# wkh923/m3pc

Hardware: AMD Instinct MI355X
Metric: MPC plan-steps/sec (N=1024, H=16, hopper-medium-v2); independent plan steps, 3 in flight (higher is better)
Workload: dtype bf16; 1 GPU; hopper-medium-v2 shapes (S=11,A=3) rtg_guiding N=1024 H=16 T=32 bf16 candidate pass + fp32 policy pass + fp32 re-score (arg-max and multinomial draw certified under the calibrated bound delta, 8.4 candidates re-scored on average); 3 independent plan steps in flight (policy pass / candidate pass / re-score of neighbouring steps on different streams); window resident in HBM; candidates_per_gpu=1024, global_candidates=1024, horizon=16, traj_length=32, steps_in_flight=3, settle_steps=24, parallelism=1 GPU

## Files before the change

include/m3pc_hip_debug.h:

```cpp
#ifndef M3PC_HIP_DEBUG_H
#define M3PC_HIP_DEBUG_H

#ifdef __cplusplus
extern "C" {
#endif

int m3pc_debug_gemm(int dtype, const void* A, const void* Wt, const float* bias, const float* res, void* C, int M, int N,
                    int K, int gelu, int f32out, int variant, void* stream);
typedef struct m3pc_debug_gemm_args {
    int dtype;
    const void* A;
    int lda;
    int amap[3];
    const void* W;
    int ldw;
    int M, N, K;
    const float* bias;
    const float* rowtab;
    int rt_mod, rt_ld;
    int gelu;
    const float* res;
    int ldr;
    void* C;
    int f32out;
// ... 553 lines not shown
    const float* grad;
    long long grad_floats;
    float* exp_avg;
    float* exp_avg_sq;
    long long state_floats;
    const long long* steps_in;
    long long* steps_out;
    int write_bf16;
    double lr_t, weight_decay, beta1, beta2, eps;
    void* stream;
    int* n_blocks;
} m3pc_debug_mtm_adamw_args;
int m3pc_debug_mtm_adamw(const m3pc_debug_mtm_adamw_args* a);
int m3pc_debug_stamp_log(m3pc_handle* h, int cap, long long* out, int* n_logged);
int m3pc_debug_step_streams_created(m3pc_handle* h);
int m3pc_debug_xcc_probe(int* out, int n_blocks, void* stream);

#ifdef __cplusplus
}
#endif
#endif
```

m3pc_amd/csrc/elementwise.hip:

```cpp
#include "device_util.h"

namespace m3pc {

#ifdef M3PC_LAB
thread_local int g_ew_picked = 0;
#endif

__global__ __launch_bounds__(256) void embed_kernel(EmbedP p) {
    const long long row = blockIdx.x;
    const int b = (int)(row / p.L), j = (int)(row % p.L);
    const int2 kt = p.tokmap[j];
    const int key = kt.x, t = kt.y;
    const int D = p.feat[key];
    const float* x = p.tok[key] + (long long)b * p.bstride[key] + (p.widx ? (long long)p.widx[b] * p.wstride[key] : 0) + (long long)t * D;
    __shared__ float xs[32];
    if (threadIdx.x < D) {
        float v = x[threadIdx.x];
        if (p.normalize[key]) v = (v - p.mean[key][threadIdx.x]) / p.stdv[key][threadIdx.x];
        xs[threadIdx.x] = v;
    }
    __syncthreads();
    const float* WT = p.WT[key];
    const float* E = p.E[key] + (long long)t * p.d;
    float* out = p.X + row * p.d;
// ... 104 lines not shown
                for (int i = 0; i < NV; ++i) {
                    const float c0 = x[i].x - mean, c1 = x[i].y - mean, c2 = x[i].z - mean, c3 = x[i].w - mean;
                    q += (c0 * c0 + c1 * c1) + (c2 * c2 + c3 * c3);
                }
                const float rstd = rsqrtf(wave_sum(q) / (float)d + 1e-5f);
#pragma unroll
                for (int i = 0; i < NV; ++i) {
                    y[i].x = (x[i].x - mean) * rstd * gv[i].x + bv[i].x;
                    y[i].y = (x[i].y - mean) * rstd * gv[i].y + bv[i].y;
                    y[i].z = (x[i].z - mean) * rstd * gv[i].z + bv[i].z;
                    y[i].w = (x[i].w - mean) * rstd * gv[i].w + bv[i].w;
                }
            }
        }
        const long long row = (long long)b * p.L + j;
        if (!(indep && p.x_first_only && b > 0)) {
            if (p.Xb) {
                const long long xrow = p.x_compact ? block_res_row_xb((int)row, p.L, p.n_indep) : row;
#pragma unroll
                for (int i = 0; i < NV; ++i) {
                    bf16x4 o;
                    o[0] = (bf16_t)x[i].x;
                    o[1] = (bf16_t)x[i].y;
                    o[2] = (bf16_t)x[i].z;
                    o[3] = (bf16_t)x[i].w;
                    stream_store(o, (bf16x4*)(p.Xb + xrow * d + (i * 64 + lane) * 4));
                }
            } else {
#pragma unroll
                for (int i = 0; i < NV; ++i) *(float4*)(p.X + row * d + (i * 64 + lane) * 4) = x[i];
            }
        }
        if (!p.ln_g) continue;
        if (p.Hf) {
#pragma unroll
            for (int i = 0; i < NV; ++i) *(float4*)(p.Hf + row * d + (i * 64 + lane) * 4) = y[i];
        }
        if (p.Hb) {
            bf16_t* dst;
            if (p.n_sh == 0)
                dst = p.Hb + row * d;
            else if (j >= p.n_sh)
                dst = p.Hb + ((long long)b * n_own + (j - p.n_sh)) * d;
            else if (b == 0)
                dst = p.Hb_sh + (long long)j * d;
            else
                continue;
#pragma unroll
            for (int i = 0; i < NV; ++i) {
                bf16x4 o;
                o[0] = (bf16_t)y[i].x;
                o[1] = (bf16_t)y[i].y;
                o[2] = (bf16_t)y[i].z;
                o[3] = (bf16_t)y[i].w;
                stream_store(o, (bf16x4*)(dst + (i * 64 + lane) * 4));
            }
        }
    }
}
// ... 851 lines not shown
```

m3pc_amd/csrc/kernels.h:

```cpp
#pragma once
#include <hip/hip_runtime.h>
#include <stdint.h>

#ifdef M3PC_LAB
#define M3PC_ENV(name) getenv(name)
#else
#define M3PC_ENV(name) ((const char*)nullptr)
#endif

namespace m3pc {

typedef __bf16 bf16_t;

enum DType { DT_F32 = 0, DT_BF16 = 1, DT_X3 = 2 };

static inline size_t dtype_size(int dt) { return dt == DT_F32 ? 4 : 2; }

#ifndef M3PC_STREAM_AUX
#define M3PC_STREAM_AUX 0
#endif
template <typename V>
__device__ __forceinline__ V stream_load(const V* p) { return M3PC_STREAM_AUX ? __builtin_nontemporal_load(p) : *p; }
template <typename V>
__device__ __forceinline__ void stream_store(V v, V* p) {
// ... 245 lines not shown
    const float* E[4];
    int feat[4];
    const int2* tokmap;
    int batch, L, d, T;
    float* X;
    bf16_t* Xb;
    const float* ln_g;
    const float* ln_b;
    float* Hf;
    bf16_t* Hb;
    int n_indep;
    int x_first_only;
    int x_compact;
    int n_sh;
    bf16_t* Hb_sh;
};
void launch_embed(const EmbedP& p, hipStream_t st);

struct GatherP {
    const float* Xe;
    long long xe_bstride;
    const float* table;
    const int* rowsrc;
    int rows_per_batch, batch, d;
    float* out;
    bf16_t* outb;
};
void launch_gather_rows(const GatherP& p, hipStream_t st);

struct HeadOutP {
// ... 246 lines not shown
```

m3pc_amd/csrc/m3pc.hip:

```cpp
#include "m3pc_internal.h"
#include "mtm_loss.h"

namespace m3pc {
thread_local char g_err[512] = "";
int fail(int code, const char* fmt, ...) {
    va_list ap;
    va_start(ap, fmt);
    vsnprintf(g_err, sizeof(g_err), fmt, ap);
    va_end(ap);
    return code;
}
}

namespace {

int find_tensor(const m3pc_named_tensor* list, int n, const std::string& name) {
    for (int i = 0; i < n; ++i)
        if (list[i].name && name == list[i].name) return i;
    return -1;
}


}

// ... 64 lines not shown
        }
        if (is_dirty("mask_token_dict." + kn))
            HIPCHK(hipMemcpyAsync(h->mask_tokens + (size_t)k * d, W(h, "mask_token_dict." + kn).f, d * sizeof(float),
                                  hipMemcpyDeviceToDevice, st));
    }
    bool dec_dirty = pos_dirty;
    for (const std::string& nme : dirty)
        if (nme.rfind("decoder", 0) == 0 || nme.rfind("mask_token_dict", 0) == 0) dec_dirty = true;
    if (dec_dirty) {
        invalidate_tables(h);
        ls[3] = 1;
    }
    for (int sl = 0; sl < M3PC_SLOTS; ++sl) {
        h->slot[sl].policy_valid = false;
        h->slot[sl].n_windows = 0;
    }
    return 0;
}
}

#pragma GCC visibility push(default)
extern "C" {

const char* m3pc_last_error(void) { return g_err; }
int m3pc_abi_version(void) { return M3PC_ABI_VERSION; }

int m3pc_create(const m3pc_dims* dims, int device, m3pc_handle** out) {
    if (!dims || !out) return fail(M3PC_EINVAL, "null argument");
    const m3pc_dims& D = *dims;
    if (D.n_embd % 64 || D.n_embd > 1024 || D.n_head <= 0 || D.n_embd % D.n_head)
// ... 164 lines not shown
        hipFree(h->Edec[k]);
        hipFree(h->tok_mean[k]);
        hipFree(h->tok_std[k]);
    }
    hipFree(h->mask_tokens);
    mtm_loss_free(h);
    free_ws(h->base);
    for (int par = 0; par < 2; ++par) {
        free_ws(h->chain[par]);
        free_ws(h->pchain[par]);
    }
    for (int s = 0; s < M3PC_SLOTS; ++s) {
        hipFree(h->slot[s].loc);
        hipFree(h->slot[s].sd);
        hipFree(h->slot[s].rtok);
    }
    void* bufs[] = {h->sel_scratch, h->d_topk, h->er_top, h->sa_buf, h->sa_chain[0], h->sa_chain[1], h->c_om, h->c_os, h->goal_ws,
                    h->refine_noise, h->refine_scores, h->refine_elites, h->refine_widx};
    for (int s = 0; s < M3PC_SLOTS; ++s) {
        void* cb[] = {h->cert_list[s], h->cert_b[s], h->cert_f[s], h->cert_stats[s], h->cert_f32[s], h->cert_top1[s]};
        for (void* b : cb)
            if (b) hipFree(b);
        for (int i = 0; i < 4; ++i)
            if (h->step_ev[s][i]) hipEventDestroy(h->step_ev[s][i]);
    }
    if (h->ev_excl) hipEventDestroy(h->ev_excl);
    if (h->step_chain_own)
        for (int i = 0; i < 2; ++i)
            if (h->step_chain[i]) hipStreamDestroy(h->step_chain[i]);
    if (h->cert_host) hipHostFree(h->cert_host);
// ... 80 lines not shown
    if (!h || !out4) return fail(M3PC_EINVAL, "null argument");
    for (int i = 0; i < 4; ++i) out4[i] = h->load_stats[i];
    return 0;
}

int m3pc_set_tokenizer(m3pc_handle* h, int key, const float* mean, const float* std_, int dim, int normalize) {
    if (!h || key < 0 || key > 3 || !mean || !std_) return fail(M3PC_EINVAL, "bad argument");
    if (dim != h->feat[key]) return fail(M3PC_EINVAL, "tokenizer '%s' has dim %d, expected %d", KEYN[key], dim, h->feat[key]);
    HIPCHK(hipSetDevice(h->device));
    HIPCHK(hipMemcpy(h->tok_mean[key], mean, dim * sizeof(float), hipMemcpyHostToDevice));
    HIPCHK(hipMemcpy(h->tok_std[key], std_, dim * sizeof(float), hipMemcpyHostToDevice));
    h->h_mean[key].assign(mean, mean + dim);
    h->h_std[key].assign(std_, std_ + dim);
    h->tok_norm[key] = normalize ? 1 : 0;
    h->tok_set[key] = true;
    return 0;
}

int m3pc_set_critic(m3pc_handle* h, const m3pc_named_tensor* tensors, int n, const float* obs_mean, const float* obs_std,
                    void* stream) {
    if (!h || !tensors || !obs_mean || !obs_std) return fail(M3PC_EINVAL, "null argument");
    if (h->dm.critic_hidden <= 0) return fail(M3PC_EINVAL, "handle was created without a critic");
    hipStream_t st = (hipStream_t)stream;
    HIPCHK(hipSetDevice(h->device));
    HIPCHK(hipStreamSynchronize(st));
    const int Hd = h->dm.critic_hidden, SA = h->S + h->A;
    auto fetch = [&](const std::string& name, long long numel, std::vector<float>& out) -> int {
        const int i = find_tensor(tensors, n, name);
        if (i < 0) return fail(M3PC_EINVAL, "critic state_dict is missing '%s'", name.c_str());
        if (tensors[i].numel != numel) return fail(M3PC_EINVAL, "'%s' has %lld elements, expected %lld", name.c_str(), tensors[i].numel, numel);
// ... 254 lines not shown
    if (a->mode < 0 || a->mode > 2) return fail(M3PC_EINVAL, "bad mode %d", a->mode);
    if (!precision_ok(a->precision)) return fail(M3PC_EINVAL, "bad precision %d", a->precision);
    if (a->slot < 0 || a->slot >= M3PC_SLOTS) return fail(M3PC_EINVAL, "slot %d outside [0, %d)", a->slot, M3PC_SLOTS);
    if (a->flags & ~(M3PC_PLAN_DEFER_JOIN | M3PC_PLAN_PRUNED_POLICY))
        return fail(M3PC_EINVAL, "unknown m3pc_plan_args::flags 0x%x (is the caller's structure the ABI v%d one?)", a->flags, M3PC_ABI_VERSION);
    if (need_critic && a->mode != M3PC_MODE_RTG && !h->critic_set) return fail(M3PC_ESTATE, "critic weights not set");
    HIPCHK(hipSetDevice(h->device));
    bind_slot(h, a->slot);
    return 0;
}

int m3pc_policy_pass(m3pc_handle* h, const m3pc_plan_args* a, const float* states, const float* actions, const float* rewards,
                     float* loc, float* std_, void* stream) {
    if (!h || !a || !states || !actions || !rewards) return fail(M3PC_EINVAL, "null argument");
    CHK(plan_check(h, a, false));
    hipStream_t st = (hipStream_t)stream;
    const int T = h->T, hh = a->horizon, idx = T - hh;
    if (a->returns) {
        launch_tokenize(a->returns, a->returns_f64, h->rtok, T, 1, h->tok_mean[M3PC_RETURNS], h->tok_std[M3PC_RETURNS],
                        h->tok_norm[M3PC_RETURNS], st);
    } else {
        double rt = a->rtg;
        if (h->tok_norm[M3PC_RETURNS]) rt = (rt - (double)h->h_mean[M3PC_RETURNS][0]) / (double)h->h_std[M3PC_RETURNS][0];
        launch_fill(h->rtok, (float)rt, T, st);
    }
    Plan* pl = nullptr;
    CHK(get_mask_plan(h, 0, idx, &pl));
    TokIn in;
    memset(&in, 0, sizeof(in));
    in.ptr[M3PC_STATES] = states;
// ... 98 lines not shown
        sp.n_begin = a->n_begin + c0;
        sp.n_count = cnt;
        sp.cand = h->base.cand + (size_t)c0 * T * h->A;
        sp.sample_actions = sample_actions + (size_t)c0 * hh * h->A;
        if (c0 == 0) {
            sp.loc_out = loc;
            sp.sd_out = std_;
        }
        launch_sample(sp, s);
    };

    const int dt = pass_dt(a->precision);
    X3Scope x3(h, a->precision == M3PC_PREC_BF16X3);
    const int n = a->n_count;
    h->slot_join_n[a->slot] = 0;
    if (h->two_stream && dt == DT_BF16 && n >= 512 && (long long)n * (2 * T - hh + 1) > 256 * 128) {
        std::vector<int> parts;
        if (!h->stream_split.empty()) {
            int left = n;
            for (int v : h->stream_split)
                if (v > 0 && v < left && parts.size() + 1 < h->auxs.size() + 1) {
                    parts.push_back(v);
                    left -= v;
                }
            parts.push_back(left);
        } else {
            int n0 = ((n / 2 + 127) / 128) * 128;
            parts = {n0, n - n0};
        }
        const bool defer = (a->flags & M3PC_PLAN_DEFER_JOIN) != 0 && !h->prof_serial && parts.size() <= 4;
// ... 44 lines not shown
    for (int i = 0; i < h->slot_join_n[slot]; ++i) HIPCHK(hipStreamWaitEvent((hipStream_t)stream, h->slot_join[slot][i], 0));
    h->slot_join_n[slot] = 0;
    return 0;
}

int m3pc_plan_step(m3pc_handle* h, const m3pc_plan_args* a, const float* states, const float* actions, const float* rewards,
                   const float* eps, float* loc, float* std_, float* sample_actions, float* expect_return,
                   float* pred_rewards, float* pred_boot, void* stream) {
    if (!h || !a || !states || !actions || !rewards || !eps || !sample_actions || !expect_return)
        return fail(M3PC_EINVAL, "null argument");
    if (a->mode >= 0 && a->mode <= 2 && a->mode != M3PC_MODE_RTG && !h->critic_set) return fail(M3PC_ESTATE, "critic weights not set");
    if (a->n_count < 1 || a->n_begin < 0 || a->n_begin + a->n_count > a->n_total)
        return fail(M3PC_EINVAL, "candidate range [%d,+%d) outside n_total=%d", a->n_begin, a->n_count, a->n_total);
    if (a->n_count > h->dm.max_candidates) return fail(M3PC_ENOMEM, "n_count %d > max_candidates %d", a->n_count, h->dm.max_candidates);
    CHK(m3pc_policy_pass(h, a, states, actions, rewards, nullptr, nullptr, stream));
    return m3pc_candidate_pass(h, a, states, actions, rewards, eps, loc, std_, sample_actions, expect_return, pred_rewards,
                               pred_boot, stream);
}

static int fill_rtok(m3pc_handle* h, const double* rtg, int n_windows, hipStream_t st) {
    for (int w = 0; w < n_windows; ++w) {
        double rt = rtg[w];
        if (h->tok_norm[M3PC_RETURNS]) rt = (rt - (double)h->h_mean[M3PC_RETURNS][0]) / (double)h->h_std[M3PC_RETURNS][0];
        launch_fill(h->rtok + (size_t)w * h->T, (float)rt, h->T, st);
    }
    return 0;
}

int m3pc_score_actions(m3pc_handle* h, const m3pc_plan_args* a, int n_windows, const float* states, const float* actions,
                       const float* rewards, const float* cand, const int* window_index, float* expect_return,
// ... 64 lines not shown
    in.normalize[M3PC_ACTIONS] = h->tok_norm[M3PC_ACTIONS];
    in.ptr[M3PC_REWARDS] = rewards;
    in.bstride[M3PC_REWARDS] = T;
    in.normalize[M3PC_REWARDS] = h->tok_norm[M3PC_REWARDS];
    in.ptr[M3PC_RETURNS] = h->rtok;
    in.bstride[M3PC_RETURNS] = T;
    h->allow_splitk = true;
    {
        WsScope ws(h, true, true, a->slot);
        const int rc = forward_impl(h, pl, in, E, nullptr, nullptr, nullptr, h->loc, h->sd, DT_F32, st);
        h->allow_splitk = false;
        if (rc) return rc;
    }
    h->slot[a->slot].policy_valid = E == 1;
    h->slot[a->slot].n_windows = E;
    if (loc) HIPCHK(hipMemcpyAsync(loc, h->loc, (size_t)E * T * A * sizeof(float), hipMemcpyDeviceToDevice, st));
    if (std_) HIPCHK(hipMemcpyAsync(std_, h->sd, (size_t)E * T * A * sizeof(float), hipMemcpyDeviceToDevice, st));
    return check_launch("policy_pass_batch");
}

int m3pc_plan_step_batch(m3pc_handle* h, const m3pc_plan_args* a, int n_windows, const float* states, const float* actions,
                         const float* rewards, const double* rtg, const float* eps, const int* window_index, float* loc,
                         float* std_, float* sample_actions, float* expect_return, void* stream) {
    if (!h || !a || !states || !actions || !rewards || !rtg || !eps || !window_index || !sample_actions || !expect_return)
        return fail(M3PC_EINVAL, "null argument");
    const int T = h->T, E = n_windows, N = a->n_total;
    if (!precision_ok(a->precision)) return fail(M3PC_EINVAL, "bad precision %d", a->precision);
    if (E >= 1 && (N < 1 || (long long)E * N > h->dm.max_candidates))
        return fail(M3PC_ENOMEM, "n_windows * n_total = %lld > max_candidates %d", (long long)E * N, h->dm.max_candidates);
    if (a->mode >= 0 && a->mode <= 2 && a->mode != M3PC_MODE_RTG && !h->critic_set) return fail(M3PC_ESTATE, "critic weights not set");
// ... 513 lines not shown
```

m3pc_amd/csrc/m3pc_certified.hip:

```cpp
#include <atomic>
#include <chrono>

#include "m3pc_internal.h"

namespace m3pc {
int cert_check_args(const m3pc_plan_args* a, const char* who) {
    if (a->n_total < 1 || a->n_total > 16384) return fail(M3PC_EINVAL, "%s: n_total %d outside [1, 16384]", who, a->n_total);
    if (a->n_begin != 0 || a->n_count != a->n_total)
        return fail(M3PC_EINVAL, "%s plans on one rank: candidates [%d,+%d) are not all n_total=%d", who, a->n_begin, a->n_count, a->n_total);
    if (!precision_ok(a->precision)) return fail(M3PC_EINVAL, "bad precision %d", a->precision);
    if (a->slot < 0 || a->slot >= M3PC_SLOTS) return fail(M3PC_EINVAL, "slot %d outside [0, %d)", a->slot, M3PC_SLOTS);
    return 0;
}
bool cert_any_begun(const m3pc_handle* h) {
    for (int s = 0; s < M3PC_SLOTS; ++s)
        if (h->cstep[s].begun) return true;
    return false;
}
}

#pragma GCC visibility push(default)
extern "C" {

static int cert_wait_blocks(const volatile float* hs, const float* dev, const float* seq, int n, int n_device, hipStream_t st, float* out) {
// ... 233 lines not shown
    if (with_eval && !(eval_tol > 0.f)) return fail(M3PC_EINVAL, "%s: eval_tol must be > 0 (+inf: report only)", who);
    if (cert_any_begun(h)) return fail(M3PC_ESTATE, "%s with a pipelined step begun (m3pc_plan_step_certified_end first)", who);
    memset(rec, 0, sizeof(*rec));
    if (with_eval) {
        memset(erec, 0, sizeof(*erec));
        if (a->precision != M3PC_PREC_FP32) CHK(eval_host_setup(h));
    }
    CertStep& S = h->cstep[a->slot];
    cert_fill(S, a, c, states, actions, rewards, eps, expo, sample_actions, scores_low, merged, list, p, eval_action, argmax, sample_idx,
              sample_action, (hipStream_t)stream, false, with_eval ? eval_tol : 0.f);

    m3pc_plan_args pa = *a;
    pa.flags = a->flags & M3PC_PLAN_PRUNED_POLICY;
    pa.window = 0;
    CHK(m3pc_policy_pass(h, &pa, states, actions, rewards, nullptr, nullptr, stream));
    pa.flags = 0;
    CHK(m3pc_candidate_pass(h, &pa, states, actions, rewards, eps, loc, std_, sample_actions, scores_low, nullptr, nullptr, stream));
    CHK(cert_first_pass(h, S));
    return cert_resolve_step(h, S, rec, with_eval ? erec : nullptr);
}

int m3pc_plan_step_certified(m3pc_handle* h, const m3pc_plan_args* a, const m3pc_cert_args* c, const float* states, const float* actions,
                             const float* rewards, const float* eps, const float* expo, float* loc, float* std_, float* sample_actions,
                             float* scores_low, float* merged, int* list, float* p, float* eval_action, int* argmax, int* sample_idx,
                             float* sample_action, m3pc_cert_record* rec, void* stream) {
    return cert_step_serial(h, a, c, states, actions, rewards, eps, expo, loc, std_, sample_actions, scores_low, merged, list, p, eval_action,
                            argmax, sample_idx, sample_action, rec, false, 0.f, nullptr, stream, "m3pc_plan_step_certified");
}

int m3pc_plan_step_certified_eval(m3pc_handle* h, const m3pc_plan_args* a, const m3pc_cert_args* c, const float* states,
// ... 66 lines not shown
    CertStep& S = h->cstep[slot];
    if (S.begun) return fail(M3PC_ESTATE, "%s: the step in slot %d has not been ended", who, slot);
    HIPCHK(hipSetDevice(h->device));
    CHK(step_setup(h));
    if (with_eval && a->precision != M3PC_PREC_FP32) CHK(eval_host_setup(h));
    hipStream_t st = (hipStream_t)stream, chain = h->step_chain[slot & 1];
    hipEvent_t* ev = h->step_ev[slot];
    if (!(a->flags & M3PC_PLAN_INPUTS_READY)) {
        HIPCHK(hipEventRecord(ev[0], st));
        HIPCHK(hipStreamWaitEvent(chain, ev[0], 0));
    }
    m3pc_plan_args pa = *a;
    pa.flags = a->flags & M3PC_PLAN_PRUNED_POLICY;
    pa.window = 0;
    CHK(m3pc_policy_pass(h, &pa, states, actions, rewards, nullptr, nullptr, chain));
    HIPCHK(hipEventRecord(ev[1], chain));
    for (;;) {
        int o = -1;
        for (int s = 0; s < M3PC_SLOTS; ++s)
            if ((s & 1) == (slot & 1) && h->cstep[s].begun && h->cstep[s].tail_pending && (o < 0 || h->cstep[s].order < h->cstep[o].order))
                o = s;
        if (o < 0) break;
        CHK(step_enqueue_tail(h, o));
    }
    HIPCHK(hipStreamWaitEvent(st, ev[1], 0));
    if (h->excl_valid) HIPCHK(hipStreamWaitEvent(st, h->ev_excl, 0));
    if (h->cand_last_slot >= 0) HIPCHK(hipStreamWaitEvent(st, h->step_ev[h->cand_last_slot][2], 0));
    pa.flags = M3PC_PLAN_DEFER_JOIN;
    CHK(m3pc_candidate_pass(h, &pa, states, actions, rewards, eps, loc, std_, sample_actions, scores_low, nullptr, nullptr, stream));
    HIPCHK(hipEventRecord(ev[2], st));
// ... 435 lines not shown
```

m3pc_amd/csrc/m3pc_debug.hip:

```cpp
#include "m3pc_internal.h"
#include "mtm_grad.h"
#include "iql.h"
#include "mtm_opt.h"

#include <vector>

#pragma GCC visibility push(default)
extern "C" {

int m3pc_debug_step_streams_created(m3pc_handle* h) { return h ? h->step_streams_created : -1; }
int m3pc_debug_gemm(int dtype, const void* A, const void* Wt, const float* bias, const float* res, void* C, int M, int N,
                    int K, int gelu, int f32out, int variant, void* stream) {
    static const int ldpad = M3PC_ENV("M3PC_DEBUG_LDPAD") ? atoi(M3PC_ENV("M3PC_DEBUG_LDPAD")) : 0;
    GemmP p = gemm_basic(A, K + ldpad, Wt, K + ldpad, M, N, K, bias);
    p.a_padded = 0;
    p.gelu = gelu;
    p.res = res;
    p.ldr = N;
    p.variant = variant;
    if (dtype == DT_BF16 && !f32out)
        p.Cb = (bf16_t*)C;
    else
        p.Cf = (float*)C;
    p.ldc = N;
    if (dtype != DT_BF16 && variant != 1) {
// ... 1897 lines not shown
```

m3pc_amd/csrc/m3pc_internal.h:

```cpp
#pragma once
#include <math.h>
#include <stdarg.h>
#include <stdio.h>
#include <stdlib.h>
#include <string.h>

#include <algorithm>
#include <map>
#include <mutex>
#include <memory>
#include <string>
#include <vector>

#include "../../include/m3pc_hip.h"
#ifdef M3PC_LAB
#include "../../include/m3pc_hip_debug.h"
#endif
#include "cert_resolve.h"
#include "kernels.h"
#include "mtm_batch.h"

using namespace m3pc;

namespace m3pc {
// ... 151 lines not shown
    } ls;
    hipStream_t step_chain[2] = {nullptr, nullptr};
    bool step_chain_own = false;
    int step_streams_created = 0;
    hipEvent_t step_ev[M3PC_SLOTS][4] = {};
    hipEvent_t ev_excl = nullptr;
    bool excl_valid = false;
    int cand_last_slot = -1;
    unsigned long long step_order = 0;
    struct Slot {
        float *loc = nullptr, *sd = nullptr, *rtok = nullptr;
        bool policy_valid = false;
        int n_windows = 0;
    } slot[M3PC_SLOTS];
    int cur_slot = 0;
    struct Base {
        float *X = nullptr, *Y = nullptr, *EncOut = nullptr, *G = nullptr, *cand = nullptr, *pred[2] = {nullptr, nullptr},
              *qv = nullptr, *splitk_ws = nullptr;
        char *Hn = nullptr, *QKV = nullptr, *O = nullptr, *F = nullptr, *Z = nullptr;
        long long splitk_ws_bytes = 0;
        float* head_part = nullptr;
        int* head_ticket = nullptr;
        int head_rows = 0;
        long long R = 0;
        int max_cand = 0;
    } base, chain[2], pchain[2];
    Base* cur = nullptr;
    bool two_stream = true;
    bool allow_splitk = true;
    bool x3 = false;
// ... 320 lines not shown
    g.rowsrc = rowsrc;
    g.rows_per_batch = rows_per_batch;
    g.batch = batch;
    g.d = h->d;
    return g;
}

struct PassSwitches {
    bool no_block_fused;
    bool no_block_split;
    bool no_qkv_fused;
    bool no_fused_anything;
    bool no_prune1;
    bool no_bf16_residual;
    bool no_shared_xb;
    bool no_kv_fused;
    bool no_mix_prefix;
    bool no_head_fused;
    bool no_head_out_mfma;
    bool no_head_f32_fused;
    bool no_group;
};
inline const PassSwitches& pass_switches() {
    static const PassSwitches s = [] {
        auto on = [](const char* v) { return v != nullptr; };
        PassSwitches w{};
        w.no_block_fused = on(M3PC_ENV("M3PC_NO_BLOCK_FUSED"));
        w.no_block_split = on(M3PC_ENV("M3PC_NO_BLOCK_SPLIT"));
        w.no_qkv_fused = on(M3PC_ENV("M3PC_NO_QKV_FUSED"));
        w.no_fused_anything = w.no_block_fused || w.no_qkv_fused;
        w.no_prune1 = on(M3PC_ENV("M3PC_NO_PRUNE1"));
        w.no_bf16_residual = on(M3PC_ENV("M3PC_NO_BF16_RESIDUAL"));
        w.no_shared_xb = on(M3PC_ENV("M3PC_NO_SHARED_XB"));
        w.no_kv_fused = on(M3PC_ENV("M3PC_NO_KV_FUSED")) || w.no_block_fused;
        w.no_mix_prefix = on(M3PC_ENV("M3PC_NO_MIX_PREFIX"));
        w.no_head_fused = on(M3PC_ENV("M3PC_NO_HEAD_FUSED"));
        w.no_head_out_mfma = on(M3PC_ENV("M3PC_NO_HEAD_OUT_MFMA"));
        const bool no_f32_direct = on(M3PC_ENV("M3PC_NO_F32_DIRECT"));
        w.no_head_f32_fused = on(M3PC_ENV("M3PC_NO_HEAD_F32_FUSED")) || no_f32_direct;
        w.no_group = on(M3PC_ENV("M3PC_NO_GEMM_GROUP")) || no_f32_direct || on(M3PC_ENV("M3PC_GEMM_VARIANT"));
        return w;
    }();
    return s;
}

constexpr long long FUSED_MIN_ROWS = 96 * 128;
constexpr long long SPLIT_MIN_ROWS = 16 * 128;

struct PieceState {
    bool ln = true, qkv = false;
};

struct BlockArgs {
    const std::string& pfx;
    float* X;
    int batch, L;
    int n_sh = 0;
    const LnP* next_ln = nullptr;
    bool x_dead = false;
    const std::string* next_qkv = nullptr;
    bool x_bf16 = false;
    float* Xnext = nullptr;
    int res_nshared = 0;
};

struct TokIn {
    const float* ptr[4];
    long long bstride[4];
    int normalize[4];
    const int* widx = nullptr;
    long long wstride[4] = {0, 0, 0, 0};
};

enum { TAIL_HEADS = 0, TAIL_X = 1 };

int get_plan(m3pc_handle* h, const unsigned char* const masks[4], Plan** out);
int get_mask_plan(m3pc_handle* h, int kind, int idx, Plan** out);
int ensure_edec(m3pc_handle* h, Plan* pl, hipStream_t st);
// ... 9 lines not shown
int run_encoder(m3pc_handle* h, Plan* pl, const TokIn& in, int batch, int dt, hipStream_t st, bool bf16_out_only = false,
                int n_indep = 0, int layer_from = 0, int layer_to = 1 << 30, PieceState* ln_state = nullptr);
void dec_embed(m3pc_handle* h, int k, const void* Zop, RowMap amap, float* Yout, RowMap cmap, int M, int mod, int dt,
               hipStream_t st, const float* table = nullptr);
int run_decoder_full(m3pc_handle* h, const void* Zop, int batch, int dt, hipStream_t st);
int run_head(m3pc_handle* h, int k, const float* Ysrc, RowMap xmap, int rows, float* out, int ldy, bool detok, int dt,
             hipStream_t st);
int run_head_tail(m3pc_handle* h, int k, const void* ln_rows, int rows, float* out, int ldy, bool detok, int dt, hipStream_t st);
int forward_impl(m3pc_handle* h, Plan* pl, const TokIn& in, int batch, float* out_states, float* out_rewards,
                 float* out_returns, float* out_mu, float* out_std, int dt, hipStream_t st);
int pruned_decoder(m3pc_handle* h, Plan* pl, Plan::Query& q, SharedTables& tb, int n, int dt, hipStream_t st, int tail,
                   float** xrows);
int candidate_pass(m3pc_handle* h, const m3pc_plan_args* a, const float* states, const float* rewards, int n,
                   const float* sample_actions, float* expect_return, float* pred_rewards, float* pred_boot, int dt,
                   hipStream_t st, const int* widx = nullptr, int stage_from = 0, int stage_to = 1 << 30, PieceState* ln_state = nullptr);

}
```

m3pc_amd/csrc/m3pc_passes.hip:

```cpp
#include "m3pc_internal.h"

namespace m3pc {

struct TailRes {
    const float* rows = nullptr;
    const float* table = nullptr;
    int mod = 0;
    int nu = 0;
};

static bool chain_tail(m3pc_handle* h, const std::string& pfx, int rows, int dt, hipStream_t st, const TailRes& res, float* Xout,
                       const LnP* next_ln) {
    const int d = h->d, ff = h->ff;
    GemmP p = gemm_basic(h->O, d, Wop(h, pfx + ".self_attn.out_proj.weight", dt), d, rows, d, d, W(h, pfx + ".self_attn.out_proj.bias").f);
    if (res.table) {
        p.rowtab = res.table;
        p.rt_mod = res.mod;
        p.rt_ld = d;
    } else {
        p.res = res.rows;
        p.ldr = d;
    }
    gemm_out(p, DT_F32, Xout, d);
    const LnP ln = ln_rows(h, Xout, rows, W(h, pfx + ".norm2.weight").f, W(h, pfx + ".norm2.bias").f, h->Hn, dt);
// ... 87 lines not shown
        b.stamp_block = 37;
    }
    bool ok;
    {
        GemmTimer t(h, st, 2.0 * rows * ((double)d * d + 2.0 * d * h->ff + extra), dt, 1);
        ok = launch_block_fused(b, st);
    }
    if (ok && form == TAIL_SPLIT) launch_block_split_reduce(r, st);
    return ok;
}

static bool tail_fuses_ln(const LnP* next_ln, const float* Xout, int rows) {
    return next_ln && next_ln->Yb && !next_ln->Yf && !next_ln->g2 && next_ln->X == Xout && next_ln->xmap.rpg == 0 && next_ln->rows == rows;
}

static void shared_rows_attention(m3pc_handle* h, const BlockArgs& a, int dt, hipStream_t st) {
    const int d = h->d, n_sh = a.n_sh, n_own = a.L - n_sh;
    const size_t es = dtype_size(dt);
    char* hn_sh = (char*)h->Hn + (size_t)a.batch * n_own * d * es;
    char* qkv_sh = (char*)h->QKV + (size_t)a.batch * n_own * 3 * d * es;
    const void* w = Wop(h, a.pfx + ".self_attn.in_proj_weight", dt);
    const float* bias = W(h, a.pfx + ".self_attn.in_proj_bias").f;
    GemmP p = gemm_basic(h->Hn, d, w, d, a.batch * n_own, 3 * d, d, bias);
    gemm_out(p, dt, h->QKV, 3 * d);
    gemm(h, p, dt, st);
    p = gemm_basic(hn_sh, d, w, d, n_sh, 3 * d, d, bias);
    gemm_out(p, dt, qkv_sh, 3 * d);
    gemm(h, p, dt, st);
    AttnP at = attn_basic(h, a.batch, a.L);
    const char* q = (const char*)h->QKV;
    at.Q = q;
    at.q_bstride = (long long)n_own * 3 * d;
    at.ldq = 3 * d;
    at.Lq = n_own;
    at.orow1 = n_sh;
    at.Q2 = qkv_sh;
    at.ldq2 = 3 * d;
    at.Lq2 = n_sh;
    at.orow2 = 0;
    at.K1 = q + (size_t)d * es;
    at.V1 = q + (size_t)2 * d * es;
    at.kv1_bstride = (long long)n_own * 3 * d;
    at.ldkv1 = 3 * d;
// ... 31 lines not shown
        if (!ln1_done && !qkv_done) launch_layernorm(ln, st);
        if (!qkv_done) gemm(h, pqkv, dt, st);
        AttnP at = attn_basic(h, a.batch, a.L);
        const char* q = (const char*)h->QKV;
        at.Q = q;
        at.q_bstride = (long long)a.L * 3 * d;
        at.ldq = 3 * d;
        at.Lq = a.L;
        at.K1 = q + (size_t)d * dtype_size(dt);
        at.V1 = q + (size_t)2 * d * dtype_size(dt);
        at.kv1_bstride = (long long)a.L * 3 * d;
        at.ldkv1 = 3 * d;
        at.L1 = a.L;
        launch_attention(at, dt, st);
    }
    if (a.x_bf16 && !ln1_done && !qkv_done) return fail(M3PC_EINVAL, "%s: norm1 of a bf16 residual stream has no kernel", pfx.c_str());
    const TailForm form = tail_form(h, pfx, rows, dt);
    TailRes res;
    res.rows = a.X;
    float* const Xout = a.Xnext ? a.Xnext : a.X;
    if (form != TAIL_CHAIN) {
        BlockP b{};
        const bool fuse_ln = tail_fuses_ln(a.next_ln, Xout, rows);
        const bool fuse_qkv = form == TAIL_FULL && fuse_ln && a.next_qkv && !pass_switches().no_qkv_fused &&
                              a.next_ln->Yb == (bf16_t*)h->Hn && (size_t)rows * 3 * d * 2 < 0x7fffffffull;
        if (a.x_bf16 && !(fuse_ln && (fuse_qkv || a.x_dead)))
            return fail(M3PC_EINVAL, "%s: a bf16 residual stream needs the consumer of the block output inside the tail", pfx.c_str());
        if (a.res_nshared > 0) {
            b.res_L = a.L;
            b.res_nshared = a.res_nshared;
// ... 31 lines not shown
int run_encoder(m3pc_handle* h, Plan* pl, const TokIn& in, int batch, int dt, hipStream_t st, bool bf16_out_only,
                int n_indep, int layer_from, int layer_to, PieceState* ln_state) {
    const PassSwitches& sw = pass_switches();
    const int Le = pl->Le, d = h->d, nl = h->dm.n_enc_layer;
    int n_sh = 0;
    if (dt == DT_BF16 && batch >= 64 && d % 256 == 0 && d <= 1024 && n_indep >= 32 && !sw.no_prune1) n_sh = (n_indep / 32) * 32;
    bool xb16 = dt == DT_BF16 && bf16_out_only && !sw.no_bf16_residual && !sw.no_fused_anything && block_fused_supported(d, h->ff) &&
                (double)batch * Le * h->pass_scale >= (double)FUSED_MIN_ROWS && (size_t)batch * Le * 3 * d * 2 < 0x7fffffffull &&
                (unsigned long long)batch * Le * d * 2 < 0x80000000ull;
    for (int i = 0; i < nl && xb16; ++i) xb16 = h->wstream.count("encoder.layers." + std::to_string(i)) != 0;
    const long long xc_rows = (long long)n_indep + (long long)batch * (Le - n_indep);
    const bool xb_shared = xb16 && n_sh > 0 && !sw.no_shared_xb && n_indep < Le &&
                           (long long)batch * Le + xc_rows <= (long long)batch * 4 * h->T &&
                           (h->X - h->cur->X) / d + (long long)batch * 2 * h->T <= h->R;
    bf16_t* const Xc = (bf16_t*)h->X + (size_t)batch * Le * d;
    if (layer_from <= 0) {
        EmbedP e{};
        e.n_indep = n_indep;
        e.n_sh = n_sh;
        e.Hb_sh = n_sh ? (bf16_t*)((char*)h->Hn + (size_t)batch * (Le - n_sh) * d * 2) : nullptr;
        for (int k = 0; k < 4; ++k) {
            e.tok[k] = in.ptr[k];
            e.bstride[k] = in.bstride[k];
            e.wstride[k] = in.wstride[k];
            e.normalize[k] = in.normalize[k];
            e.mean[k] = h->tok_mean[k];
            e.stdv[k] = h->tok_std[k];
            e.WT[k] = h->WT[k];
            e.E[k] = h->Eenc[k];
            e.feat[k] = h->feat[k];
        }
        e.x_first_only = e.x_compact = xb_shared ? 1 : 0;
        if (xb16) e.Xb = xb_shared ? Xc : (bf16_t*)h->X;
        e.widx = in.widx;
        e.tokmap = pl->d_tokmap;
// ... 7 lines not shown
        if (dt == DT_BF16)
            e.Hb = (bf16_t*)h->Hn;
        else
            e.Hf = (float*)h->Hn;
        launch_embed(e, st);
    }
    const LnP ln = ln_rows(h, h->X, batch * Le, W(h, "encoder.norm.weight").f, W(h, "encoder.norm.bias").f,
                           bf16_out_only ? (void*)h->Z : (void*)h->EncOut, bf16_out_only ? DT_BF16 : DT_F32);
    PieceState ps = layer_from <= 0 || !ln_state ? PieceState{} : *ln_state;
    for (int i = layer_from > 0 ? layer_from : 0; i < nl && i < layer_to; ++i) {
        const std::string pfx = "encoder.layers." + std::to_string(i), nq = "encoder.layers." + std::to_string(i + 1);
        LnP nxt = ln;
        if (i + 1 < nl) nxt = ln_rows(h, h->X, batch * Le, W(h, nq + ".norm1.weight").f, W(h, nq + ".norm1.bias").f, h->Hn, dt);
        BlockArgs b{pfx, h->X, batch, Le};
        b.n_sh = i == 0 ? n_sh : 0;
        b.next_ln = &nxt;
        b.x_dead = i + 1 == nl && bf16_out_only;
        b.next_qkv = i + 1 < nl ? &nq : nullptr;
        b.x_bf16 = xb16;
        if (xb_shared && i == 0) {
            b.X = (float*)Xc;
            b.Xnext = h->X;
            b.res_nshared = n_indep;
        }
        CHK(run_block(h, b, dt, st, ps));
    }
    if (ln_state) *ln_state = ps;
    if (layer_to >= nl && !ps.ln) launch_layernorm(ln, st);
    return check_launch("encoder");
}

static GemmP dec_embed_p(m3pc_handle* h, int k, const void* Zop, RowMap amap, float* Yout, RowMap cmap, int M, int mod, int dt,
                         const float* table) {
    const int d = h->d;
    GemmP p = gemm_basic(Zop, d, Wop(h, std::string("decoder_embed_dict.") + KEYN[k] + ".weight", dt), d, M, d, d, nullptr);
    p.amap = amap;
    p.cmap = cmap;
    p.rowtab = table ? table : h->Edec[k];
    p.rt_mod = mod;
    p.rt_ld = d;
    gemm_out(p, DT_F32, Yout, d);
    return p;
}
void dec_embed(m3pc_handle* h, int k, const void* Zop, RowMap amap, float* Yout, RowMap cmap, int M, int mod, int dt,
// ... 443 lines not shown
    const int Le = pl->Le, nq = q.nq;
    if ((long long)n * Le > h->R || (long long)n * nq > h->R) return fail(M3PC_ENOMEM, "n_count %d exceeds workspace", n);

    TokIn in{};
    in.ptr[M3PC_STATES] = states;
    in.normalize[M3PC_STATES] = h->tok_norm[M3PC_STATES];
    in.ptr[M3PC_ACTIONS] = h->cand;
    in.bstride[M3PC_ACTIONS] = (long long)T * h->A;
    in.normalize[M3PC_ACTIONS] = h->tok_norm[M3PC_ACTIONS];
    in.ptr[M3PC_REWARDS] = rewards;
    in.ptr[M3PC_RETURNS] = h->rtok;
    in.widx = widx;
    in.wstride[M3PC_STATES] = (long long)T * h->S;
    in.wstride[M3PC_REWARDS] = T;
    const int nl_enc = h->dm.n_enc_layer;
    if (stage_from < nl_enc) CHK(run_encoder(h, pl, in, n, dt, st, dt == DT_BF16, widx ? 0 : (idx + 1) + idx, stage_from, stage_to, ln_state));
    if (stage_to <= nl_enc) return check_launch("candidate_pass");

    CHK(pruned_decoder(h, pl, q, tb, n, dt, st, TAIL_HEADS, nullptr));
    const float* rw;
    const float* boot;
    float boot_scale;
    if (a->mode == M3PC_MODE_RTG) {
        rw = h->pred[0];
        boot = h->pred[1];
        boot_scale = 1000.0f;
    } else {
        if (!h->critic_set) return fail(M3PC_ESTATE, "critic weights not set");
        CriticP c{};
        c.states = h->pred[0];
// ... 43 lines not shown
```

Baseline: 881.4 plan-steps/s.

## Compute shared history rows' layer-0 norm and QKV once per plan step

Adds a per-slot history block: after the policy pass, a prologue embeds the shared history rows, applies layer-0 norm1 and runs their QKV projection once into a dedicated buffer. Candidate passes, including those split across two streams, then reuse these rows instead of recomputing the shared embed/norm and shared QKV GEMM each time. The cache is keyed on slot, index and input pointers and is invalidated on normalisation changes, batch policy passes and after each candidate pass. This adds a small serial prologue on the chain stream and some extra state to manage.

```diff
diff --git a/include/m3pc_hip_debug.h b/include/m3pc_hip_debug.h
--- a/include/m3pc_hip_debug.h
+++ b/include/m3pc_hip_debug.h
@@ -591,6 +591,9 @@
 int m3pc_debug_mtm_adamw(const m3pc_debug_mtm_adamw_args* a);
 int m3pc_debug_stamp_log(m3pc_handle* h, int cap, long long* out, int* n_logged);
 int m3pc_debug_step_streams_created(m3pc_handle* h);
+int m3pc_debug_layer1_head(m3pc_handle* h, const m3pc_plan_args* a, const float* states, const float* actions, const float* rewards,
+                           const float* eps, int use_block, void* hn_sh, void* qkv_sh, void* O, int* n_sh_out, int* used_block,
+                           void* stream);
 int m3pc_debug_xcc_probe(int* out, int n_blocks, void* stream);
 
 #ifdef __cplusplus
diff --git a/m3pc_amd/csrc/elementwise.hip b/m3pc_amd/csrc/elementwise.hip
--- a/m3pc_amd/csrc/elementwise.hip
+++ b/m3pc_amd/csrc/elementwise.hip
@@ -142,7 +142,7 @@
             }
         }
         const long long row = (long long)b * p.L + j;
-        if (!(indep && p.x_first_only && b > 0)) {
+        if (!p.hist_only && !(indep && p.x_first_only && b > 0)) {
             if (p.Xb) {
                 const long long xrow = p.x_compact ? block_res_row_xb((int)row, p.L, p.n_indep) : row;
 #pragma unroll
@@ -170,7 +170,7 @@
                 dst = p.Hb + row * d;
             else if (j >= p.n_sh)
                 dst = p.Hb + ((long long)b * n_own + (j - p.n_sh)) * d;
-            else if (b == 0)
+            else if (b == 0 && !p.sh_extern)
                 dst = p.Hb_sh + (long long)j * d;
             else
                 continue;
diff --git a/m3pc_amd/csrc/kernels.h b/m3pc_amd/csrc/kernels.h
--- a/m3pc_amd/csrc/kernels.h
+++ b/m3pc_amd/csrc/kernels.h
@@ -283,6 +283,8 @@
     int x_compact;
     int n_sh;
     bf16_t* Hb_sh;
+    int sh_extern;
+    int hist_only;
 };
 void launch_embed(const EmbedP& p, hipStream_t st);
 
diff --git a/m3pc_amd/csrc/m3pc.hip b/m3pc_amd/csrc/m3pc.hip
--- a/m3pc_amd/csrc/m3pc.hip
+++ b/m3pc_amd/csrc/m3pc.hip
@@ -102,6 +102,7 @@
     for (int sl = 0; sl < M3PC_SLOTS; ++sl) {
         h->slot[sl].policy_valid = false;
         h->slot[sl].n_windows = 0;
+        history_invalidate(h, sl);
     }
     return 0;
 }
@@ -296,6 +297,7 @@
         hipFree(h->slot[s].loc);
         hipFree(h->slot[s].sd);
         hipFree(h->slot[s].rtok);
+        if (h->hist[s].buf) hipFree(h->hist[s].buf);
     }
     void* bufs[] = {h->sel_scratch, h->d_topk, h->er_top, h->sa_buf, h->sa_chain[0], h->sa_chain[1], h->c_om, h->c_os, h->goal_ws,
                     h->refine_noise, h->refine_scores, h->refine_elites, h->refine_widx};
@@ -406,6 +408,7 @@
     h->h_std[key].assign(std_, std_ + dim);
     h->tok_norm[key] = normalize ? 1 : 0;
     h->tok_set[key] = true;
+    for (int sl = 0; sl < M3PC_SLOTS; ++sl) history_invalidate(h, sl);
     return 0;
 }
 
@@ -690,6 +693,7 @@
                      float* loc, float* std_, void* stream) {
     if (!h || !a || !states || !actions || !rewards) return fail(M3PC_EINVAL, "null argument");
     CHK(plan_check(h, a, false));
+    history_invalidate(h, a->slot);
     hipStream_t st = (hipStream_t)stream;
     const int T = h->T, hh = a->horizon, idx = T - hh;
     if (a->returns) {
@@ -818,6 +822,18 @@
     X3Scope x3(h, a->precision == M3PC_PREC_BF16X3);
     const int n = a->n_count;
     h->slot_join_n[a->slot] = 0;
+    struct HistScope {
+        m3pc_handle* h;
+        int slot;
+        ~HistScope() {
+            h->hist_use = nullptr;
+            history_invalidate(h, slot);
+        }
+    } hist_scope{h, a->slot};
+    const m3pc_handle::HistBlock& hb = h->hist[a->slot];
+    if (hb.valid && a->precision == M3PC_PREC_BF16 && a->window == 0 && h->slot[a->slot].n_windows == 1 && hb.idx == idx &&
+        hb.states == states && hb.actions == actions)
+        h->hist_use = &hb;
     if (h->two_stream && dt == DT_BF16 && n >= 512 && (long long)n * (2 * T - hh + 1) > 256 * 128) {
         std::vector<int> parts;
         if (!h->stream_split.empty()) {
@@ -892,6 +908,7 @@
         return fail(M3PC_EINVAL, "candidate range [%d,+%d) outside n_total=%d", a->n_begin, a->n_count, a->n_total);
     if (a->n_count > h->dm.max_candidates) return fail(M3PC_ENOMEM, "n_count %d > max_candidates %d", a->n_count, h->dm.max_candidates);
     CHK(m3pc_policy_pass(h, a, states, actions, rewards, nullptr, nullptr, stream));
+    CHK(history_prologue(h, a, states, actions, (hipStream_t)stream));
     return m3pc_candidate_pass(h, a, states, actions, rewards, eps, loc, std_, sample_actions, expect_return, pred_rewards,
                                pred_boot, stream);
 }
@@ -986,6 +1003,7 @@
     }
     h->slot[a->slot].policy_valid = E == 1;
     h->slot[a->slot].n_windows = E;
+    history_invalidate(h, a->slot);
     if (loc) HIPCHK(hipMemcpyAsync(loc, h->loc, (size_t)E * T * A * sizeof(float), hipMemcpyDeviceToDevice, st));
     if (std_) HIPCHK(hipMemcpyAsync(std_, h->sd, (size_t)E * T * A * sizeof(float), hipMemcpyDeviceToDevice, st));
     return check_launch("policy_pass_batch");
diff --git a/m3pc_amd/csrc/m3pc_certified.hip b/m3pc_amd/csrc/m3pc_certified.hip
--- a/m3pc_amd/csrc/m3pc_certified.hip
+++ b/m3pc_amd/csrc/m3pc_certified.hip
@@ -271,6 +271,7 @@
     pa.flags = a->flags & M3PC_PLAN_PRUNED_POLICY;
     pa.window = 0;
     CHK(m3pc_policy_pass(h, &pa, states, actions, rewards, nullptr, nullptr, stream));
+    CHK(history_prologue(h, &pa, states, actions, (hipStream_t)stream));
     pa.flags = 0;
     CHK(m3pc_candidate_pass(h, &pa, states, actions, rewards, eps, loc, std_, sample_actions, scores_low, nullptr, nullptr, stream));
     CHK(cert_first_pass(h, S));
@@ -367,6 +368,7 @@
     pa.flags = a->flags & M3PC_PLAN_PRUNED_POLICY;
     pa.window = 0;
     CHK(m3pc_policy_pass(h, &pa, states, actions, rewards, nullptr, nullptr, chain));
+    CHK(history_prologue(h, &pa, states, actions, chain));
     HIPCHK(hipEventRecord(ev[1], chain));
     for (;;) {
         int o = -1;
diff --git a/m3pc_amd/csrc/m3pc_debug.hip b/m3pc_amd/csrc/m3pc_debug.hip
--- a/m3pc_amd/csrc/m3pc_debug.hip
+++ b/m3pc_amd/csrc/m3pc_debug.hip
@@ -9,6 +9,47 @@
 extern "C" {
 
 int m3pc_debug_step_streams_created(m3pc_handle* h) { return h ? h->step_streams_created : -1; }
+int m3pc_debug_layer1_head(m3pc_handle* h, const m3pc_plan_args* a, const float* states, const float* actions, const float* rewards,
+                           const float* eps, int use_block, void* hn_sh, void* qkv_sh, void* O, int* n_sh_out, int* used_block,
+                           void* stream) {
+    if (!h || !a || !states || !actions || !rewards || !eps) return fail(M3PC_EINVAL, "debug_layer1_head: null argument");
+    if (a->slot < 0 || a->slot >= M3PC_SLOTS || a->horizon < 1 || a->horizon > h->T || a->n_count < 1 || a->n_count > h->dm.max_candidates)
+        return fail(M3PC_EINVAL, "debug_layer1_head: slot / horizon / n_count");
+    if (a->precision != M3PC_PREC_BF16) return fail(M3PC_EINVAL, "debug_layer1_head: a bf16 pass (the rows copied out are bf16)");
+    hipStream_t st = (hipStream_t)stream;
+    m3pc_plan_args pa = *a;
+    pa.flags = 0;
+    pa.window = 0;
+    if (use_block)
+        CHK(history_prologue(h, &pa, states, actions, st));
+    else
+        history_invalidate(h, pa.slot);
+    float *sa = nullptr, *er = nullptr;
+    CHK(dmalloc(&sa, (size_t)pa.n_count * pa.horizon * h->A));
+    CHK(dmalloc(&er, (size_t)pa.n_count));
+    h->lab_l1 = m3pc_handle::LabLayer1{};
+    h->lab_l1.on = true;
+    int rc = m3pc_candidate_pass(h, &pa, states, actions, rewards, eps, nullptr, nullptr, sa, er, nullptr, nullptr, stream);
+    const m3pc_handle::LabLayer1 l1 = h->lab_l1;
+    h->lab_l1 = m3pc_handle::LabLayer1{};
+    const size_t d = (size_t)h->d, Le = (size_t)(h->T - pa.horizon + 1) + h->T;
+    if (rc == 0 && l1.n_sh > 0 && hn_sh && hipMemcpyAsync(hn_sh, l1.hn_sh, l1.n_sh * d * 2, hipMemcpyDeviceToDevice, st) != hipSuccess)
+        rc = fail(M3PC_EHIP, "debug_layer1_head: copy of the norm1 rows");
+    if (rc == 0 && l1.n_sh > 0 && qkv_sh && hipMemcpyAsync(qkv_sh, l1.qkv_sh, l1.n_sh * 3 * d * 2, hipMemcpyDeviceToDevice, st) != hipSuccess)
+        rc = fail(M3PC_EHIP, "debug_layer1_head: copy of the Q|K|V rows");
+    size_t c0 = 0;
+    for (const auto& part : l1.O) {
+        if (rc == 0 && O && hipMemcpyAsync((char*)O + c0 * Le * d * 2, part.first, (size_t)part.second * Le * d * 2, hipMemcpyDeviceToDevice, st) != hipSuccess)
+            rc = fail(M3PC_EHIP, "debug_layer1_head: copy of the attention rows");
+        c0 += (size_t)part.second;
+    }
+    if (hipStreamSynchronize(st) != hipSuccess && rc == 0) rc = fail(M3PC_EHIP, "debug_layer1_head: synchronise");
+    hipFree(sa);
+    hipFree(er);
+    if (n_sh_out) *n_sh_out = l1.n_sh;
+    if (used_block) *used_block = l1.block ? 1 : 0;
+    return rc;
+}
 int m3pc_debug_gemm(int dtype, const void* A, const void* Wt, const float* bias, const float* res, void* C, int M, int N,
                     int K, int gelu, int f32out, int variant, void* stream) {
     static const int ldpad = M3PC_ENV("M3PC_DEBUG_LDPAD") ? atoi(M3PC_ENV("M3PC_DEBUG_LDPAD")) : 0;
diff --git a/m3pc_amd/csrc/m3pc_internal.h b/m3pc_amd/csrc/m3pc_internal.h
--- a/m3pc_amd/csrc/m3pc_internal.h
+++ b/m3pc_amd/csrc/m3pc_internal.h
@@ -189,6 +189,19 @@
         int n_windows = 0;
     } slot[M3PC_SLOTS];
     int cur_slot = 0;
+    struct HistBlock {
+        bf16_t* buf = nullptr;
+        bool valid = false;
+        int idx = -1, n_sh = 0;
+        const float *states = nullptr, *actions = nullptr;
+    } hist[M3PC_SLOTS];
+    const HistBlock* hist_use = nullptr;
+    struct LabLayer1 {
+        bool on = false, block = false;
+        const void *hn_sh = nullptr, *qkv_sh = nullptr;
+        int n_sh = 0;
+        std::vector<std::pair<const void*, int>> O;
+    } lab_l1;
     struct Base {
         float *X = nullptr, *Y = nullptr, *EncOut = nullptr, *G = nullptr, *cand = nullptr, *pred[2] = {nullptr, nullptr},
               *qv = nullptr, *splitk_ws = nullptr;
@@ -539,6 +552,7 @@
     bool no_prune1;
     bool no_bf16_residual;
     bool no_shared_xb;
+    bool no_history_once;
     bool no_kv_fused;
     bool no_mix_prefix;
     bool no_head_fused;
@@ -557,6 +571,7 @@
         w.no_prune1 = on(M3PC_ENV("M3PC_NO_PRUNE1"));
         w.no_bf16_residual = on(M3PC_ENV("M3PC_NO_BF16_RESIDUAL"));
         w.no_shared_xb = on(M3PC_ENV("M3PC_NO_SHARED_XB"));
+        w.no_history_once = on(M3PC_ENV("M3PC_NO_HISTORY_ONCE"));
         w.no_kv_fused = on(M3PC_ENV("M3PC_NO_KV_FUSED")) || w.no_block_fused;
         w.no_mix_prefix = on(M3PC_ENV("M3PC_NO_MIX_PREFIX"));
         w.no_head_fused = on(M3PC_ENV("M3PC_NO_HEAD_FUSED"));
@@ -587,6 +602,7 @@
     bool x_bf16 = false;
     float* Xnext = nullptr;
     int res_nshared = 0;
+    const m3pc_handle::HistBlock* hist = nullptr;
 };
 
 struct TokIn {
@@ -626,5 +642,7 @@
 int candidate_pass(m3pc_handle* h, const m3pc_plan_args* a, const float* states, const float* rewards, int n,
                    const float* sample_actions, float* expect_return, float* pred_rewards, float* pred_boot, int dt,
                    hipStream_t st, const int* widx = nullptr, int stage_from = 0, int stage_to = 1 << 30, PieceState* ln_state = nullptr);
-
-}
+int history_prologue(m3pc_handle* h, const m3pc_plan_args* a, const float* states, const float* actions, hipStream_t st);
+inline void history_invalidate(m3pc_handle* h, int slot) { h->hist[slot].valid = false; }
+
+}
diff --git a/m3pc_amd/csrc/m3pc_passes.hip b/m3pc_amd/csrc/m3pc_passes.hip
--- a/m3pc_amd/csrc/m3pc_passes.hip
+++ b/m3pc_amd/csrc/m3pc_passes.hip
@@ -125,19 +125,39 @@
     return next_ln && next_ln->Yb && !next_ln->Yf && !next_ln->g2 && next_ln->X == Xout && next_ln->xmap.rpg == 0 && next_ln->rows == rows;
 }
 
+static void shared_qkv_gemm(m3pc_handle* h, const std::string& pfx, const void* hn_sh, void* qkv_sh, int n_sh, int dt, hipStream_t st) {
+    const int d = h->d;
+    GemmP p = gemm_basic(hn_sh, d, Wop(h, pfx + ".self_attn.in_proj_weight", dt), d, n_sh, 3 * d, d, W(h, pfx + ".self_attn.in_proj_bias").f);
+    gemm_out(p, dt, qkv_sh, 3 * d);
+    gemm(h, p, dt, st);
+}
+static bf16_t* hist_hn(const m3pc_handle::HistBlock& hb) { return hb.buf; }
+static bf16_t* hist_qkv(const m3pc_handle* h, const m3pc_handle::HistBlock& hb) { return hb.buf + (size_t)2 * h->T * h->d; }
+
 static void shared_rows_attention(m3pc_handle* h, const BlockArgs& a, int dt, hipStream_t st) {
     const int d = h->d, n_sh = a.n_sh, n_own = a.L - n_sh;
     const size_t es = dtype_size(dt);
-    char* hn_sh = (char*)h->Hn + (size_t)a.batch * n_own * d * es;
-    char* qkv_sh = (char*)h->QKV + (size_t)a.batch * n_own * 3 * d * es;
     const void* w = Wop(h, a.pfx + ".self_attn.in_proj_weight", dt);
     const float* bias = W(h, a.pfx + ".self_attn.in_proj_bias").f;
     GemmP p = gemm_basic(h->Hn, d, w, d, a.batch * n_own, 3 * d, d, bias);
     gemm_out(p, dt, h->QKV, 3 * d);
     gemm(h, p, dt, st);
-    p = gemm_basic(hn_sh, d, w, d, n_sh, 3 * d, d, bias);
-    gemm_out(p, dt, qkv_sh, 3 * d);
-    gemm(h, p, dt, st);
+    const char *hn_sh, *qkv_sh;
+    if (a.hist) {
+        hn_sh = (const char*)hist_hn(*a.hist);
+        qkv_sh = (const char*)hist_qkv(h, *a.hist);
+    } else {
+        char* const own_sh = (char*)h->QKV + (size_t)a.batch * n_own * 3 * d * es;
+        hn_sh = (const char*)h->Hn + (size_t)a.batch * n_own * d * es;
+        shared_qkv_gemm(h, a.pfx, hn_sh, own_sh, n_sh, dt, st);
+        qkv_sh = own_sh;
+    }
+    if (h->lab_l1.on) {
+        h->lab_l1.hn_sh = hn_sh;
+        h->lab_l1.qkv_sh = qkv_sh;
+        h->lab_l1.n_sh = n_sh;
+        h->lab_l1.block = a.hist != nullptr;
+    }
     AttnP at = attn_basic(h, a.batch, a.L);
     const char* q = (const char*)h->QKV;
     at.Q = q;
@@ -199,6 +219,10 @@
         at.L1 = a.L;
         launch_attention(at, dt, st);
     }
+    if (h->lab_l1.on) {
+        h->lab_l1.O.push_back({h->O, a.batch});
+        return check_launch(pfx.c_str());
+    }
     if (a.x_bf16 && !ln1_done && !qkv_done) return fail(M3PC_EINVAL, "%s: norm1 of a bf16 residual stream has no kernel", pfx.c_str());
     const TailForm form = tail_form(h, pfx, rows, dt);
     TailRes res;
@@ -260,11 +284,13 @@
                            (long long)batch * Le + xc_rows <= (long long)batch * 4 * h->T &&
                            (h->X - h->cur->X) / d + (long long)batch * 2 * h->T <= h->R;
     bf16_t* const Xc = (bf16_t*)h->X + (size_t)batch * Le * d;
+    const m3pc_handle::HistBlock* const hist = h->hist_use && n_sh > 0 && n_sh == h->hist_use->n_sh ? h->hist_use : nullptr;
     if (layer_from <= 0) {
         EmbedP e{};
         e.n_indep = n_indep;
         e.n_sh = n_sh;
         e.Hb_sh = n_sh ? (bf16_t*)((char*)h->Hn + (size_t)batch * (Le - n_sh) * d * 2) : nullptr;
+        e.sh_extern = hist ? 1 : 0;
         for (int k = 0; k < 4; ++k) {
             e.tok[k] = in.ptr[k];
             e.bstride[k] = in.bstride[k];
@@ -302,6 +328,7 @@
         if (i + 1 < nl) nxt = ln_rows(h, h->X, batch * Le, W(h, nq + ".norm1.weight").f, W(h, nq + ".norm1.bias").f, h->Hn, dt);
         BlockArgs b{pfx, h->X, batch, Le};
         b.n_sh = i == 0 ? n_sh : 0;
+        b.hist = i == 0 ? hist : nullptr;
         b.next_ln = &nxt;
         b.x_dead = i + 1 == nl && bf16_out_only;
         b.next_qkv = i + 1 < nl ? &nq : nullptr;
@@ -316,6 +343,56 @@
     if (ln_state) *ln_state = ps;
     if (layer_to >= nl && !ps.ln) launch_layernorm(ln, st);
     return check_launch("encoder");
+}
+
+int history_prologue(m3pc_handle* h, const m3pc_plan_args* a, const float* states, const float* actions, hipStream_t st) {
+    if (!h || !a || a->slot < 0 || a->slot >= M3PC_SLOTS) return 0;
+    m3pc_handle::HistBlock& hb = h->hist[a->slot];
+    hb.valid = false;
+    const PassSwitches& sw = pass_switches();
+    const int T = h->T, d = h->d;
+    if (sw.no_history_once || sw.no_prune1 || a->precision != M3PC_PREC_BF16 || a->n_count < 64 || !states || !actions ||
+        a->horizon < 1 || a->horizon > T || d % 256 != 0 || d > 1024 || !h->weights_loaded || !h->tok_set[M3PC_STATES] ||
+        !h->tok_set[M3PC_ACTIONS])
+        return 0;
+    const int idx = T - a->horizon, n_indep = (idx + 1) + idx, n_sh = (n_indep / 32) * 32;
+    if (n_sh == 0) return 0;
+    HIPCHK(hipSetDevice(h->device));
+    Plan* pl = nullptr;
+    CHK(get_mask_plan(h, 1, idx, &pl));
+    if (!hb.buf) CHK(dmalloc(&hb.buf, ((size_t)2 * T * 4 + 127) * d));
+    EmbedP e{};
+    e.hist_only = 1;
+    e.n_indep = e.n_sh = e.L = n_sh;
+    e.batch = 1;
+    e.d = d;
+    e.T = T;
+    e.tok[M3PC_STATES] = states;
+    e.tok[M3PC_ACTIONS] = actions;
+    for (int k = 0; k < 4; ++k) {
+        e.normalize[k] = k == M3PC_STATES || k == M3PC_ACTIONS ? h->tok_norm[k] : 0;
+        e.mean[k] = h->tok_mean[k];
+        e.stdv[k] = h->tok_std[k];
+        e.WT[k] = h->WT[k];
+        e.E[k] = h->Eenc[k];
+        e.feat[k] = h->feat[k];
+    }
+    e.tokmap = pl->d_tokmap;
+    e.ln_g = W(h, "encoder.layers.0.norm1.weight").f;
+    e.ln_b = W(h, "encoder.layers.0.norm1.bias").f;
+    e.Hb = e.Hb_sh = hist_hn(hb);
+    launch_embed(e, st);
+    const bool splitk = h->allow_splitk;
+    h->allow_splitk = false;
+    shared_qkv_gemm(h, "encoder.layers.0", hist_hn(hb), hist_qkv(h, hb), n_sh, DT_BF16, st);
+    h->allow_splitk = splitk;
+    CHK(check_launch("history_prologue"));
+    hb.idx = idx;
+    hb.n_sh = n_sh;
+    hb.states = states;
+    hb.actions = actions;
+    hb.valid = true;
+    return 0;
 }
 
 static GemmP dec_embed_p(m3pc_handle* h, int k, const void* Zop, RowMap amap, float* Yout, RowMap cmap, int M, int mod, int dt,
@@ -789,6 +866,10 @@
     in.wstride[M3PC_STATES] = (long long)T * h->S;
     in.wstride[M3PC_REWARDS] = T;
     const int nl_enc = h->dm.n_enc_layer;
+    if (h->lab_l1.on) {
+        if (stage_from > 0) return 0;
+        stage_to = 1;
+    }
     if (stage_from < nl_enc) CHK(run_encoder(h, pl, in, n, dt, st, dt == DT_BF16, widx ? 0 : (idx + 1) + idx, stage_from, stage_to, ln_state));
     if (stage_to <= nl_enc) return check_launch("candidate_pass");
 
```

Result: no change. 878.4 plan-steps/s (-0.3%).
